# NVlabs/intrinsic3d

Measured on NVIDIA H100. Metric: gauss_newton_iterations_per_sec, higher is better.
Workload: dtype f32

## Files before the change

### intrinsic3d_b200/csrc/i3d_engine.cu

```cuda
#include <cuda_runtime.h>
#include <dlfcn.h>

#include <algorithm>
#include <chrono>
#include <climits>
#include <cmath>
#include <cstdarg>
#include <cstdio>
#include <cstdlib>
#include <cstring>
#include <string>
#include <vector>

#include "../../include/i3d_c_api.h"
#include "i3d_kernels.cuh"
#include "i3d_lighting.cuh"
#include "i3d_recolor.cuh"
#include "i3d_gridops.cuh"
#include "i3d_host.h"
#include "i3d_frames.h"
#include "i3d_fusion.h"
#include "i3d_mesh.h"
#include "i3d_render.h"
#include "i3d_track.h"
// ... 432 lines not shown

int check_frame_limit(I3DEngine* e, int F, int K)
{
    int optin = 0;
    CK(cudaDeviceGetAttribute(&optin, cudaDevAttrMaxSharedMemoryPerBlockOptin, e->device));
    cudaFuncAttributes fa_acc{}, fa_app{};
    CK(cudaFuncGetAttributes(&fa_acc, k_eg_accum));
    CK(cudaFuncGetAttributes(&fa_app, k_eg_apply));
    const size_t lim = static_cast<size_t>(optin);
    auto fits = [&](int f) { return fa_acc.sharedSizeBytes + accum_smem_bytes(f, K) <= lim && fa_app.sharedSizeBytes + apply_smem_bytes(f, K) <= lim; };
    if (fits(F)) return 0;
    int fmax = 0;
    while (fits(fmax + 1)) ++fmax;
    return fail(e, "i3d_gn_iteration: %d frames at K = %d observations need %zu bytes of shared memory per block in k_eg_accum (device limit %d): "
                   "at most %d frames at K = %d", F, K, fa_acc.sharedSizeBytes + accum_smem_bytes(F, K), optin, fmax, K);
}

void launch_eg_apply(I3DEngine* e, const GridView& g, const RegView& rv, const EgRows& rows, const SolveVecs& sv)
{
    if (rows.n_active == 0) return;
    Timer kt(e->timing, e->stream, "k_eg_apply");
    pdl_launch(e, k_eg_apply, blocks_for(rows.n_active), kThreads, apply_smem_bytes(e->F, rows.K), g, rows, rv, sv, sv.ps, e->ctl.p, e->site(SITE_EG_APPLY));
}

void launch_operator(I3DEngine* e, const GridView& g, const RegView& rv, const EgRows& rows, const SolveVecs& sv, const Shard& sh, const float* vin,
                     float dmin, float dmax, int is_cg_iteration)
{
    launch_eg_apply(e, g, rv, rows, sv);
    {
        Timer kt(e->timing, e->stream, "k_op_partial", 1);
        pdl_launch(e, k_op_partial, blocks_for(static_cast<size_t>((e->held_count() + 3) / 4)), kThreads, 0,
            g, rv, sv, sh, e->held_count(), vin, sv.ps, e->type_w.p, dmin, dmax, e->ctl.p, e->site(SITE_OP_POST), e->site(SITE_EG_APPLY).out, is_cg_iteration);
    }
    if (e->world > 1)
    {
        Timer kt(e->timing, e->stream, "exchange", 1);
        exchange(e, sv.qg, nullptr, sv.qg + 2 * e->n, 6 * e->F + 9, e->site(SITE_OP_POST).out, 1, 1, is_cg_iteration ? EPI_OPERATOR_CG : -1);
    }
}

bool plan_cg_step(I3DEngine* e)
{
    if (e->step_n == e->n) return e->step_grid > 0;
    e->step_n = e->n; e->step_grid = 0;
    int sms = 0, optin = 0;
    CK(cudaDeviceGetAttribute(&sms, cudaDevAttrMultiProcessorCount, e->device));
    CK(cudaDeviceGetAttribute(&optin, cudaDevAttrMaxSharedMemoryPerBlockOptin, e->device));
    cudaFuncAttributes fa0{}, fa1{};
    CK(cudaFuncGetAttributes(&fa0, k_cg_step<false>));
    CK(cudaFuncGetAttributes(&fa1, k_cg_step<true>));
    const size_t dyn_max = static_cast<size_t>(optin) - std::max(fa0.sharedSizeBytes, fa1.sharedSizeBytes);
    CK(cudaFuncSetAttribute(k_cg_step<false>, cudaFuncAttributeMaxDynamicSharedMemorySize, static_cast<int>(dyn_max)));
    CK(cudaFuncSetAttribute(k_cg_step<true>, cudaFuncAttributeMaxDynamicSharedMemorySize, static_cast<int>(dyn_max)));
    const int64_t items = (e->n + 3) / 4;
    for (int bps = 2048 / kStepThreads; bps >= 1; --bps)
    {
        const int64_t threads = static_cast<int64_t>(bps) * sms * kStepThreads;
        const int64_t K = (items + threads - 1) / threads;
        const size_t smem = static_cast<size_t>(K) * kStepSlots * kStepThreads * sizeof(float);
        if (smem > dyn_max) break;
        int occ0 = 0, occ1 = 0;
        CK(cudaOccupancyMaxActiveBlocksPerMultiprocessor(&occ0, k_cg_step<false>, kStepThreads, smem));
        CK(cudaOccupancyMaxActiveBlocksPerMultiprocessor(&occ1, k_cg_step<true>, kStepThreads, smem));
        if (std::min(occ0, occ1) < bps) continue;
        if (static_cast<size_t>(bps) * sms + 8 > e->max_blocks) break;
        e->step_grid = static_cast<unsigned>(bps * sms); e->step_K = static_cast<int>(K); e->step_smem = smem;
        return true;
    }
    return false;
}

template <bool INIT>
void launch_cg_step(I3DEngine* e, const GridView& g, const RegView& rv, const SolveVecs& sv, float dmin, float dmax)
{
    const int64_t items = (e->n + 3) / 4;
    pdl_launch<true>(e, k_cg_step<INIT>, e->step_grid, kStepThreads, e->step_smem, g, rv, sv, items, e->step_K, e->type_w.p, e->minv.p, dmin, dmax,
                     e->ctl.p, e->site(SITE_OP_POST), e->site(SITE_EG_APPLY).out, e->site(SITE_UPDATE));
}

int gn_iteration_impl(I3DEngine* e, const I3DParams& P, I3DIterInfo& info)
{
    std::memset(&info, 0, sizeof(info));
    if (e->n <= 0) return fail(e, "i3d_gn_iteration: no grid uploaded");
    if (e->F <= 0) return fail(e, "i3d_gn_iteration: no frames uploaded");
    if (!e->have_cam) return fail(e, "i3d_gn_iteration: camera not set");
    if (!e->have_sh) return fail(e, "i3d_gn_iteration: SH coefficients not set");
    if (e->world > 1 && !e->shard_ready) return fail(e, "i3d_gn_iteration: world > 1 but i3d_set_shard was not called after the grid/frames upload");
    int K = P.num_observations;
    if (K <= 0 || K > e->F) K = e->F;
    if (K > I3D_MAX_OBS) return fail(e, "i3d_gn_iteration: num_observations (%d) exceeds I3D_MAX_OBS (%d)", K, I3D_MAX_OBS);
    if (P.lm_steps < 1) return fail(e, "i3d_gn_iteration: lm_steps < 1");
    if (P.residual_reset_period < 1) return fail(e, "i3d_gn_iteration: residual_reset_period < 1");
    if (check_frame_limit(e, e->F, K) != 0) return 1;
    e->K = K;
    e->last_params = P;
    e->timing.phases.clear(); begin_timing(e->timing, {}); e->launches = 0; e->host_syncs = 0;
    const int64_t n = e->n;
    const int F = e->F;
    const bool multi = e->world > 1;
    cudaStream_t st = e->stream;
    ensure_vectors(e);
    e->iter_dev.ensure(1);
    const Shard sh = e->shard();
    const int64_t own = sh.own_end - sh.own_begin;
    const int64_t hc = e->held_count();
    const size_t U = static_cast<size_t>(e->U());
    Timer t_total(e->timing, e->stream, "total");
    auto sync = [&]() { CK(cudaStreamSynchronize(st)); e->host_syncs += 1; };

    Timer t_sel(e->timing, e->stream, "select");
    e->flags.ensure(n);
    GridView g = e->grid_view(e->sdf, e->alb);
    pdl_launch(e, k_flags, blocks_for(static_cast<size_t>(sh.loc_end - sh.loc_begin)), kThreads, 0, g, sh, P.thres_shell, P.fix_all_albedo, e->flags.p);
    const int nscan = std::max(1, static_cast<int>((own + kScanChunk - 1) / kScanChunk));
    e->scan_counts.ensure(nscan); e->scan_total.ensure(1); e->act.ensure(n);
    pdl_launch(e, k_scan_count, nscan, kThreads, 0, own, e->flags.p + sh.own_begin, FL_ROW, e->scan_counts.p);
    pdl_launch(e, k_scan_blocks, 1, 1024, 0, nscan, e->scan_counts.p, e->scan_total.p);
    pdl_launch(e, k_scan_scatter, nscan, kThreads, 0, own, e->flags.p + sh.own_begin, FL_ROW, e->scan_counts.p, e->act.p, static_cast<int32_t>(sh.own_begin));
    const CamAccLayout lay{F};
    CK(cudaMemsetAsync(e->v_bg.p, 0, U * sizeof(float), st));
    CK(cudaMemsetAsync(e->v_cg.p, 0, U * sizeof(float), st));
    CK(cudaMemsetAsync(e->v_qg.p, 0, U * sizeof(float), st));
    CK(cudaMemsetAsync(e->v_delta.p, 0, U * sizeof(float), st));
    CK(cudaMemsetAsync(e->v_tr.p, 0, static_cast<size_t>(n) * sizeof(float), st));
    CK(cudaMemsetAsync(e->cam_acc.p, 0, lay.size() * sizeof(float), st));
    CK(cudaMemsetAsync(e->v_bgd.p, 0, U * sizeof(double), st));
    CK(cudaMemsetAsync(e->v_cgd.p, 0, U * sizeof(double), st));
    CK(cudaMemsetAsync(e->v_qgd.p, 0, U * sizeof(double), st));
    CK(cudaMemsetAsync(e->cam_accd.p, 0, lay.size() * sizeof(double), st));
    CK(cudaMemsetAsync(e->red_out.p, 0, 2 * kSiteVals * sizeof(double), st));
    e->Rt.ensure(12 * static_cast<size_t>(F));
    e->pose_ctx.ensure(F); e->pose_ctx_c.ensure(F);
    pdl_launch(e, k_pose_mats, blocks_for(F, 64), 64, 0, F, e->cam, e->Rt.p);
    pdl_launch(e, k_frame_pose, blocks_for(F, 64), 64, 0, F, e->cam, e->pose_ctx.p);
    int32_t n_active = 0;
    double hc9[9];
    CK(cudaMemcpyAsync(&n_active, e->scan_total.p, sizeof(int32_t), cudaMemcpyDeviceToHost, st));
    CK(cudaMemcpyAsync(hc9, e->cam + 6 * static_cast<size_t>(F), 9 * sizeof(double), cudaMemcpyDeviceToHost, st));
    sync();
    e->n_active = n_active;
    const int stride = (n_active + 63) & ~63;
    e->stride = stride;
    const size_t S = static_cast<size_t>(K) * stride;

    e->obs_frame.ensure(S + 1); e->obs_w.ensure(S + 1);
    if (n_active > 0)
    {
        const SelectCam sc = select_cam(e, hc9, P.occlusion_distance);
        const size_t smem = 12 * static_cast<size_t>(F) * sizeof(float);
        auto kern = (K <= 5) ? k_select_obs<5> : k_select_obs<I3D_MAX_OBS>;
        if (smem > 48 * 1024) CK(cudaFuncSetAttribute(kern, cudaFuncAttributeMaxDynamicSharedMemorySize, static_cast<int>(smem)));
        Timer kt(e->timing, e->stream, "k_select_obs");
        static const bool want_stats = std::getenv("I3D_CULL_STATS") != nullptr;
        e->cull_stats.ensure(2);
        if (want_stats) CK(cudaMemsetAsync(e->cull_stats.p, 0, 2 * sizeof(unsigned long long), st));
        const CullView cull = cull_view(e, want_stats ? e->cull_stats.p : nullptr);
        pdl_launch(e, kern, blocks_for(static_cast<size_t>(n_active)), kThreads, smem, g, e->frame_view(), e->Rt.p, sc, cull, n_active, stride, e->act.p, K,
                                                                                e->obs_frame.p, e->obs_w.p);
        if (want_stats)
        {
            unsigned long long hs[2] = {0, 0};
            CK(cudaMemcpyAsync(hs, e->cull_stats.p, sizeof(hs), cudaMemcpyDeviceToHost, st));
            CK(cudaStreamSynchronize(st));
            fprintf(stderr, "[i3d] frame culling: %llu of %llu (warp, frame) pairs visited (%.1f %%)\n", hs[0], hs[1], hs[1] ? 100.0 * hs[0] / hs[1] : 0.0);
        }
    }
    t_sel.stop();

    Timer t_build(e->timing, e->stream, "build");
    e->Jt.ensure(EgRows::kTiles * S + 1); e->Jtail.ensure(S + 1);
    e->row_frame.ensure(S + 1); e->row_res.ensure(S + 1); e->row_wraw.ensure(S + 1);
    e->ea_w.ensure(3 * static_cast<size_t>(n)); e->lap.ensure(n);
    CK(cudaFuncSetAttribute(k_eg_apply, cudaFuncAttributeMaxDynamicSharedMemorySize, static_cast<int>(apply_smem_bytes(F, K))));
    const EgRows rows = eg_rows(e);
    CamView cv{e->cam, e->pose_ctx.p, F};
    if (n_active > 0)
    {
        {
            Timer kt(e->timing, e->stream, "k_eg_build");
            launch_eg_rows<ROWS_BUILD>(e, g, cv, rows, e->obs_frame.p, e->obs_w.p);
        }
        const size_t smem = accum_smem_bytes(F, K);
        if (smem > 48 * 1024) CK(cudaFuncSetAttribute(k_eg_accum, cudaFuncAttributeMaxDynamicSharedMemorySize, static_cast<int>(smem)));
        {
            Timer kt(e->timing, e->stream, "k_eg_accum", 1);
            pdl_launch(e, k_eg_accum, blocks_for(static_cast<size_t>(n_active)), kThreads, smem, g, rows, F, e->v_bgd.p, e->v_cgd.p, e->cam_accd.p, e->site(SITE_BUILD));
        }
        pdl_launch(e, k_acc_to_float, blocks_for(std::max(U, static_cast<size_t>(lay.size()))), kThreads, 0, static_cast<int64_t>(U), lay.size(),
                   e->v_bgd.p, e->v_cgd.p, e->cam_accd.p, e->v_bg.p, e->v_cg.p, e->cam_acc.p);
    }
    const RegView rv = reg_view(e, P);
    pdl_launch(e, k_reg_build, blocks_for(static_cast<size_t>((sh.loc_end - sh.loc_begin + 3) / 4)), kThreads, 0, g, rv, sh, e->site(SITE_REG));
    {
        const double na = static_cast<double>(n_active);
        CK(cudaMemcpyAsync(e->site(SITE_BUILD).out + 3, &na, sizeof(double), cudaMemcpyHostToDevice, st));
    }
    if (multi) exchange(e, e->v_bg.p, e->v_cg.p, e->cam_acc.p, lay.size(), e->red_out.p, 2 * kSiteVals, 0);
    pdl_launch(e, k_type_weights, 1, 32, 0, e->iter_dev.p, e->site(SITE_BUILD).out, e->site(SITE_REG).out, P, n, e->type_w.p);
    if (S > 0) pdl_launch(e, k_row_weights, blocks_for(S), kThreads, 0, rows, e->type_w.p);
    SolveVecs sv = solve_vecs(e);
    pdl_launch(e, k_finish_problem, blocks_for(static_cast<size_t>((hc + 3) / 4)), kThreads, 0, g, rv, sv, sh, hc, e->type_w.p, e->cam_acc.p, P.fix_poses, P.fix_intrinsics,
                                                                              P.fix_distortion, P.gradient_tolerance, e->site(SITE_FINISH), e->cam);
    allreduce_scalars(e, e->site(SITE_FINISH).out, 3, -1, 0);
    pdl_launch(e, k_iter_finish, 1, 32, 0, e->iter_dev.p, e->site(SITE_FINISH).out, P);
    t_build.stop();
    e->have_iter = true;
    if (P.build_only)
    {
        IterDev hb{};
        CK(cudaMemcpyAsync(&hb, e->iter_dev.p, sizeof(hb), cudaMemcpyDeviceToHost, st));
        sync();
        CK(cudaGetLastError());
        info = hb.info;
        t_total.stop();
        return 0;
    }

    Timer t_solve(e->timing, e->stream, "solve");
    const float dmin = static_cast<float>(P.min_lm_diagonal), dmax = static_cast<float>(std::min(P.max_lm_diagonal, 3.0e38));
    const unsigned upd_blocks = blocks_for(static_cast<size_t>((sh.held_voxel_unknowns() + 3) / 4 + F + 2));
    auto launch_update = [&](bool init, int refresh) {
        if (init) pdl_launch(e, k_cg_update<true>, upd_blocks, kThreads, 0, sv, sh, e->minv.p, dmin, dmax, e->ctl.p, refresh, e->site(SITE_UPDATE));
        else pdl_launch(e, k_cg_update<false>, upd_blocks, kThreads, 0, sv, sh, e->minv.p, dmin, dmax, e->ctl.p, refresh, e->site(SITE_UPDATE));
    };
    const unsigned vec_blocks = blocks_for(static_cast<size_t>(hc));
    const int max_it = P.forced_cg_iterations > 0 ? P.forced_cg_iterations : P.max_linear_solver_iterations;
    const bool fused = e->pcg_fused && !multi && plan_cg_step(e);
    int enq = 0;
    bool dir_ready = false;
    auto enqueue_pcg = [&](int count) {
        for (int bidx = 0; bidx < count && enq < max_it; ++bidx)
        {
            ++enq;
            const bool refresh = (enq % P.residual_reset_period == 0);
            if (!dir_ready)
            {
                Timer kt(e->timing, e->stream, "k_cg_dir", 1);
                pdl_launch(e, k_cg_dir4, blocks_for(static_cast<size_t>((hc + 3) / 4)), kThreads, 0, sv, sh, hc, e->ctl.p);
            }
            dir_ready = false;
            if (fused && !refresh)
            {
                launch_eg_apply(e, g, rv, rows, sv);
                Timer kt(e->timing, e->stream, "k_cg_update", 1);
                launch_cg_step<false>(e, g, rv, sv, dmin, dmax);
                dir_ready = true;
                continue;
            }
            launch_operator(e, g, rv, rows, sv, sh, sv.p, dmin, dmax, 1);
            if (refresh)
            {
                pdl_launch(e, k_x_update, vec_blocks, kThreads, 0, sv, sh, hc, e->ctl.p);
                CK(cudaMemsetAsync(e->v_qg.p, 0, U * sizeof(float), st));
                pdl_launch(e, k_scale_vec, vec_blocks, kThreads, 0, sv, sh, hc, sv.x, 1.0f, sv.ps, e->ctl.p, 1);
                launch_operator(e, g, rv, rows, sv, sh, sv.x, dmin, dmax, 0);
                launch_update(false, 1);
            }
            else
            {
                Timer kt(e->timing, e->stream, "k_cg_update", 1);
                launch_update(false, 0);
            }
            if (multi) allreduce_scalars(e, e->site(SITE_UPDATE).out, 3, EPI_UPDATE, 1);
        }
    };
    auto enqueue_decision = [&]() {
        Timer t_cand(e->timing, e->stream, "candidate");
        CK(cudaMemsetAsync(e->red_out.p + SITE_CAND * kSiteVals, 0, 3 * kSiteVals * sizeof(double), st));
        pdl_launch(e, k_candidate, vec_blocks, kThreads, 0, g, sv, sh, hc, 0, e->cam, e->c_sdf, e->c_alb, e->c_cam, e->v_delta.p, e->ctl.p, e->site(SITE_CAND));
        GridView gc = e->grid_view(e->c_sdf, e->c_alb);
        pdl_launch(e, k_frame_pose, blocks_for(F, 64), 64, 0, F, e->c_cam, e->pose_ctx_c.p);
        CamView cvc{e->c_cam, e->pose_ctx_c.p, F};
        if (n_active > 0)
        {
            Timer kt(e->timing, e->stream, "k_eg_cost");
            launch_eg_rows<ROWS_COST>(e, gc, cvc, rows, nullptr, nullptr);
        }
        pdl_launch(e, k_reg_cost, blocks_for(static_cast<size_t>(own)), kThreads, 0, gc, rv, sh, e->c_sdf, e->c_alb, e->site(SITE_REG_COST));
        if (multi) allreduce_scalars(e, e->red_out.p + SITE_CAND * kSiteVals, 3 * kSiteVals, -1, 0);
        pdl_launch(e, k_lm_decide, 1, 32, 0, e->iter_dev.p, e->ctl.p, e->fail_flag.p, e->site(SITE_CAND).out, e->site(SITE_EG_COST).out,
                                      e->site(SITE_REG_COST).out, e->type_w.p, P);
    };
    IterDev h{};
    for (int it = 1; it <= P.lm_steps; ++it)
    {
        Timer t_pcg(e->timing, e->stream, "pcg");
        pdl_launch(e, k_lm_begin, 1, 32, 0, e->iter_dev.p, e->ctl.p, e->fail_flag.p, P);
        pdl_launch(e, k_cam_precond, blocks_for(static_cast<size_t>(F) + 2, 64), 64, 0, sv, e->cam_acc.p, e->type_w.p, e->ctl.p, dmin, dmax, e->minv.p, e->fail_flag.p);
        if (fused) launch_cg_step<true>(e, g, rv, sv, dmin, dmax);
        else launch_update(true, 0);
        dir_ready = fused;
        if (multi) allreduce_scalars(e, e->site(SITE_UPDATE).out, 3, EPI_UPDATE_INIT, 0);
        enq = 0;
        enqueue_pcg(P.forced_cg_iterations > 0 ? P.forced_cg_iterations : std::max(e->last_cg_iterations, e->prev_cg_iterations));
        t_pcg.stop();
        while (true)
        {
            enqueue_decision();
            CK(cudaMemcpyAsync(&h, e->iter_dev.p, sizeof(h), cudaMemcpyDeviceToHost, st));
            sync();
            CK(cudaGetLastError());
            if (!h.pcg_unfinished || h.state != LM_RUNNING) break;
            Timer t_more(e->timing, e->stream, "pcg");
            enqueue_pcg(2);
        }
        if (h.info.lm_iterations >= 1)
        {
            e->prev_cg_iterations = e->last_cg_iterations;
            e->last_cg_iterations = std::max(1, h.info.cg_iterations[std::min(h.info.lm_iterations - 1, I3D_MAX_LM_STEPS - 1)]);
        }
        if (h.state != LM_RUNNING) break;
    }
    info = h.info;
    if (h.precond_fail) e->error = "camera preconditioner block not SPD";
    if (h.state == LM_ACCEPTED)
    {
        if (multi)
// ... 1312 lines not shown
```

### intrinsic3d_b200/csrc/i3d_kernels.cuh

```cuda
#pragma once
#include <cuda_runtime.h>
#include <cooperative_groups.h>
#include <stdint.h>
#include <limits.h>
#include "i3d_math.cuh"
#include "i3d_grid.cuh"
#include "../../include/i3d_types.h"

namespace i3d
{

enum : uint8_t { FL_VALID = 1, FL_ACTIVE = 2, FL_RING = 4, FL_FREE_SDF = 8, FL_FREE_ALB = 16, FL_ES_JAC = 32, FL_ROW = 64  };

struct Shard
{
    int64_t own_begin, own_end;
    int64_t hv0, hv1;
    int cam_owner;
    int defer;
    int64_t loc_begin, loc_end;
    __device__ __forceinline__ bool owns_voxel(int64_t v) const { return v >= own_begin && v < own_end; }
    __device__ __forceinline__ bool owns_unknown(int64_t j, int64_t n) const
    {
        return j < n ? owns_voxel(j) : (j < 2 * n ? owns_voxel(j - n) : cam_owner != 0);
// ... 178 lines not shown
}

__global__ void k_flags(GridView g, Shard sh, double thres_shell, int fix_all_albedo, uint8_t* __restrict__ flags)
{
    pdl_prologue();
    const int64_t v = sh.loc_begin + blockIdx.x * static_cast<int64_t>(blockDim.x) + threadIdx.x;
    if (v >= sh.loc_end) return;
    uint8_t fl = 0;
    const bool valid = g.weight[v] > 0.0f;
    if (valid) fl |= FL_VALID;
    bool ring = true;
#pragma unroll
    for (int o = 0; o < 6; ++o)
    {
        const int32_t nb = g.nbr[static_cast<int64_t>(o) * g.n + v];
        if (nb < 0 || !(g.weight[nb] > 0.0f)) ring = false;
    }
    if (ring) fl |= FL_RING;
    const double s = g.sdf[v];
    const bool inshell = !(fabs(s) > thres_shell);
    if (valid && inshell)
    {
        float nrm[3];
        if (surface_normal_f(g, v, nrm)) { fl |= FL_ACTIVE; if (sh.owns_voxel(v)) fl |= FL_ROW; }
        if (ring) { fl |= FL_FREE_SDF; if (!fix_all_albedo) fl |= FL_FREE_ALB; }
    }
    if ((s - g.sdf0[v]) != 0.0) fl |= FL_ES_JAC;
    flags[v] = fl;
}

constexpr int kScanItems = 8;
constexpr int kScanChunk = kThreads * kScanItems;

__global__ void k_scan_count(int64_t n, const uint8_t* __restrict__ flags, uint8_t bit, int32_t* __restrict__ block_counts)
{
    pdl_prologue();
    __shared__ int smem[32];
    const int64_t base = static_cast<int64_t>(blockIdx.x) * kScanChunk;
    int c = 0;
#pragma unroll
    for (int i = 0; i < kScanItems; ++i)
    {
        const int64_t idx = base + static_cast<int64_t>(i) * kThreads + threadIdx.x;
        if (idx < n && (flags[idx] & bit)) c++;
    }
    const int lane = threadIdx.x & 31, wid = threadIdx.x >> 5;
#pragma unroll
    for (int o = 16; o > 0; o >>= 1) c += __shfl_down_sync(0xffffffffu, c, o);
    if (lane == 0) smem[wid] = c;
    __syncthreads();
    if (threadIdx.x == 0)
    {
        int s = 0;
        for (int w = 0; w < kThreads / 32; ++w) s += smem[w];
        block_counts[blockIdx.x] = s;
    }
}

__global__ void k_scan_blocks(int nblocks, int32_t* __restrict__ block_counts, int32_t* __restrict__ total)
{
    pdl_prologue();
    __shared__ int carry;
    __shared__ int wsum[32];
    if (threadIdx.x == 0) carry = 0;
    __syncthreads();
    for (int base = 0; base < nblocks; base += blockDim.x)
    {
        const int i = base + threadIdx.x;
        const int v = (i < nblocks) ? block_counts[i] : 0;
        int incl = v;
        const int lane = threadIdx.x & 31, wid = threadIdx.x >> 5;
#pragma unroll
        for (int o = 1; o < 32; o <<= 1) { const int t = __shfl_up_sync(0xffffffffu, incl, o); if (lane >= o) incl += t; }
        if (lane == 31) wsum[wid] = incl;
        __syncthreads();
        if (wid == 0)
        {
            int w = (lane < (blockDim.x >> 5)) ? wsum[lane] : 0;
#pragma unroll
            for (int o = 1; o < 32; o <<= 1) { const int t = __shfl_up_sync(0xffffffffu, w, o); if (lane >= o) w += t; }
            wsum[lane] = w;
        }
        __syncthreads();
        const int woff = (wid > 0) ? wsum[wid - 1] : 0;
        const int excl = carry + woff + incl - v;
        if (i < nblocks) block_counts[i] = excl;
        __syncthreads();
        if (threadIdx.x == blockDim.x - 1) carry = excl + v;
        __syncthreads();
    }
    if (threadIdx.x == 0) *total = carry;
}

__global__ void k_scan_scatter(int64_t n, const uint8_t* __restrict__ flags, uint8_t bit, const int32_t* __restrict__ block_offsets,
                               int32_t* __restrict__ out_list, int32_t index_offset = 0)
{
    pdl_prologue();
    __shared__ int wsum[kThreads / 32];
    const int64_t base = static_cast<int64_t>(blockIdx.x) * kScanChunk;
    int running = block_offsets[blockIdx.x];
    const int lane = threadIdx.x & 31, wid = threadIdx.x >> 5;
    for (int i = 0; i < kScanItems; ++i)
    {
        const int64_t idx = base + static_cast<int64_t>(i) * kThreads + threadIdx.x;
        const bool f = idx < n && (flags[idx] & bit);
        const unsigned bal = __ballot_sync(0xffffffffu, f);
        if (lane == 0) wsum[wid] = __popc(bal);
        __syncthreads();
        int woff = 0, tot = 0;
        for (int w = 0; w < kThreads / 32; ++w) { const int c = wsum[w]; if (w < wid) woff += c; tot += c; }
        if (f) out_list[running + woff + __popc(bal & ((1u << lane) - 1u))] = static_cast<int32_t>(idx) + index_offset;
        running += tot;
        __syncthreads();
    }
}

__global__ void k_pose_mats(int F, const double* __restrict__ poses, float* __restrict__ Rt )
{
    pdl_prologue();
    const int f = blockIdx.x * blockDim.x + threadIdx.x;
    if (f >= F) return;
    const double wx = poses[6 * f], wy = poses[6 * f + 1], wz = poses[6 * f + 2];
    const double n2 = wx * wx + wy * wy + wz * wz;
    const double angle = sqrt(n2);
    double ax = wx, ay = wy, az = wz;
    if (n2 > 0.0) { ax = wx / angle; ay = wy / angle; az = wz / angle; }
    const double s = sin(angle), c = cos(angle);
    const double sx = __dmul_rn(s, ax), sy = __dmul_rn(s, ay), sz = __dmul_rn(s, az);
    const double c1x = __dmul_rn(1.0 - c, ax), c1y = __dmul_rn(1.0 - c, ay), c1z = __dmul_rn(1.0 - c, az);
    double M[9];
    double tmp;
    tmp = __dmul_rn(c1x, ay); M[1] = tmp - sz; M[3] = tmp + sz;
    tmp = __dmul_rn(c1x, az); M[2] = tmp + sy; M[6] = tmp - sy;
    tmp = __dmul_rn(c1y, az); M[5] = tmp - sx; M[7] = tmp + sx;
    M[0] = __dadd_rn(__dmul_rn(c1x, ax), c); M[4] = __dadd_rn(__dmul_rn(c1y, ay), c); M[8] = __dadd_rn(__dmul_rn(c1z, az), c);
    float* o = Rt + 12 * f;
#pragma unroll
    for (int i = 0; i < 9; ++i) o[i] = static_cast<float>(M[i]);
    o[9] = static_cast<float>(poses[6 * f + 3]); o[10] = static_cast<float>(poses[6 * f + 4]); o[11] = static_cast<float>(poses[6 * f + 5]);
}

__global__ void k_frame_pose(int F, const double* __restrict__ poses, FramePose* __restrict__ out)
{
    pdl_prologue();
    const int f = blockIdx.x * blockDim.x + threadIdx.x;
    if (f >= F) return;
    FramePose fp;
    frame_pose_make(poses + 6 * f, &fp);
    out[f] = fp;
}

struct SelectCam { float fx, fy, cx, cy; float d[5]; int dist_zero; float occlusion; };

__device__ __forceinline__ float observation_weight(const float pt[3], const float nrm[3], const float* __restrict__ Rt, const SelectCam& cam,
                                                    const float* __restrict__ depth, int W, int H, float* pix = nullptr)
{
    float q[3];
#pragma unroll
    for (int k = 0; k < 3; ++k) q[k] = FA(FA(FA(FM(Rt[3 * k], pt[0]), FM(Rt[3 * k + 1], pt[1])), FM(Rt[3 * k + 2], pt[2])), Rt[9 + k]);
    float x = FD(q[0], q[2]);
    float y = FD(q[1], q[2]);
    if (!cam.dist_zero)
    {
        const float r2 = FA(FM(x, x), FM(y, y));
        const float r4 = FM(r2, r2);
        const float r6 = FM(r4, r2);
        const float dc = FA(FA(FA(1.0f, FM(cam.d[0], r2)), FM(cam.d[1], r4)), FM(cam.d[2], r6));
        const float xn = FA(FA(FM(x, dc), FM(FM(FM(2.0f, cam.d[3]), x), y)), FM(cam.d[4], FA(r2, FM(FM(2.0f, x), x))));
        const float yn = FA(FA(FM(y, dc), FM(FM(FM(2.0f, cam.d[4]), xn), y)), FM(cam.d[3], FA(r2, FM(FM(2.0f, y), y))));
        x = xn; y = yn;
    }
    const float pu = FA(FM(cam.fx, x), cam.cx);
    const float pv = FA(FM(cam.fy, y), cam.cy);
    if (pix) { pix[0] = pu; pix[1] = pv; }
    const float pu5 = FA(pu, 0.5f), pv5 = FA(pv, 0.5f);
    if (!(pu5 > -2147483000.0f && pu5 < 2147483000.0f && pv5 > -2147483000.0f && pv5 < 2147483000.0f)) return 0.0f;
    const int iu = __float2int_rz(pu5), iv = __float2int_rz(pv5);
    if (iu < 0 || iu >= W || iv < 0 || iv >= H) return 0.0f;
    const float d = __ldg(depth + static_cast<size_t>(iv) * W + iu);
    if (cam.occlusion > 0.0f)
    {
        if (!(d > 0.0f)) return 0.0f;
        const float sd = FS(d, q[2]);
        if (!(fabsf(sd) <= cam.occlusion)) return 0.0f;
    }
    if (d <= 0.0f) return 0.0f;
    float nc[3];
#pragma unroll
    for (int k = 0; k < 3; ++k) nc[k] = FA(FA(FM(Rt[3 * k], nrm[0]), FM(Rt[3 * k + 1], nrm[1])), FM(Rt[3 * k + 2], nrm[2]));
    float w_normal = 0.0f;
    if (!(nc[0] == 0.0f && nc[1] == 0.0f && nc[2] == 0.0f))
    {
        const float qn2 = FA(FA(FM(q[0], q[0]), FM(q[1], q[1])), FM(q[2], q[2]));
        float v0 = q[0], v1 = q[1], v2 = q[2];
        if (qn2 > 0.0f) { const float ql = __fsqrt_rn(qn2); v0 = FD(q[0], ql); v1 = FD(q[1], ql); v2 = FD(q[2], ql); }
        const float dt = FA(FA(FM(v0, nc[0]), FM(v1, nc[1])), FM(v2, nc[2]));
        w_normal = FS(1.0f, fabsf(dt));
        w_normal = (1.0f < w_normal) ? 1.0f : w_normal;
        w_normal = (w_normal < 0.0f) ? 0.0f : w_normal;
        const float div = FA(1.0f, FM(2.0f, w_normal));
        const float rk = FD(1.0f, FM(FM(div, div), div));
        w_normal = (rk < 0.001f) ? 0.001f : rk;
    }
    return w_normal;
}

struct ObsProbe { float q0, q1, q2, d; int ok; };
__device__ __forceinline__ ObsProbe obs_probe(const float pt[3], const float* __restrict__ Rt, const SelectCam& cam, const float* __restrict__ depth, int W, int H)
{
    ObsProbe o;
    float q[3];
#pragma unroll
    for (int k = 0; k < 3; ++k) q[k] = FA(FA(FA(FM(Rt[3 * k], pt[0]), FM(Rt[3 * k + 1], pt[1])), FM(Rt[3 * k + 2], pt[2])), Rt[9 + k]);
    o.q0 = q[0]; o.q1 = q[1]; o.q2 = q[2]; o.d = 0.0f; o.ok = 0;
    float x = FD(q[0], q[2]);
    float y = FD(q[1], q[2]);
    if (!cam.dist_zero)
    {
        const float r2 = FA(FM(x, x), FM(y, y));
        const float r4 = FM(r2, r2);
        const float r6 = FM(r4, r2);
        const float dc = FA(FA(FA(1.0f, FM(cam.d[0], r2)), FM(cam.d[1], r4)), FM(cam.d[2], r6));
        const float xn = FA(FA(FM(x, dc), FM(FM(FM(2.0f, cam.d[3]), x), y)), FM(cam.d[4], FA(r2, FM(FM(2.0f, x), x))));
        const float yn = FA(FA(FM(y, dc), FM(FM(FM(2.0f, cam.d[4]), xn), y)), FM(cam.d[3], FA(r2, FM(FM(2.0f, y), y))));
        x = xn; y = yn;
    }
    const float pu5 = FA(FA(FM(cam.fx, x), cam.cx), 0.5f), pv5 = FA(FA(FM(cam.fy, y), cam.cy), 0.5f);
    if (!(pu5 > -2147483000.0f && pu5 < 2147483000.0f && pv5 > -2147483000.0f && pv5 < 2147483000.0f)) return o;
    const int iu = __float2int_rz(pu5), iv = __float2int_rz(pv5);
    if (iu < 0 || iu >= W || iv < 0 || iv >= H) return o;
    o.d = __ldg(depth + static_cast<size_t>(iv) * W + iu);
    o.ok = 1;
    return o;
}
__device__ __forceinline__ float obs_finish(const ObsProbe& o, const float nrm[3], const float* __restrict__ Rt, const SelectCam& cam)
{
    if (!o.ok) return 0.0f;
    const float d = o.d;
    const float q[3] = {o.q0, o.q1, o.q2};
    if (cam.occlusion > 0.0f)
    {
        if (!(d > 0.0f)) return 0.0f;
        const float sd = FS(d, q[2]);
        if (!(fabsf(sd) <= cam.occlusion)) return 0.0f;
    }
    if (d <= 0.0f) return 0.0f;
    float nc[3];
#pragma unroll
    for (int k = 0; k < 3; ++k) nc[k] = FA(FA(FM(Rt[3 * k], nrm[0]), FM(Rt[3 * k + 1], nrm[1])), FM(Rt[3 * k + 2], nrm[2]));
    float w_normal = 0.0f;
    if (!(nc[0] == 0.0f && nc[1] == 0.0f && nc[2] == 0.0f))
    {
        const float qn2 = FA(FA(FM(q[0], q[0]), FM(q[1], q[1])), FM(q[2], q[2]));
        float v0 = q[0], v1 = q[1], v2 = q[2];
        if (qn2 > 0.0f) { const float ql = __fsqrt_rn(qn2); v0 = FD(q[0], ql); v1 = FD(q[1], ql); v2 = FD(q[2], ql); }
        const float dt = FA(FA(FM(v0, nc[0]), FM(v1, nc[1])), FM(v2, nc[2]));
        w_normal = FS(1.0f, fabsf(dt));
        w_normal = (1.0f < w_normal) ? 1.0f : w_normal;
        w_normal = (w_normal < 0.0f) ? 0.0f : w_normal;
        const float div = FA(1.0f, FM(2.0f, w_normal));
        const float rk = FD(1.0f, FM(FM(div, div), div));
        w_normal = (rk < 0.001f) ? 0.001f : rk;
    }
    return w_normal;
}

constexpr int kCullTile = 32;
constexpr int kCullMaxWords = 16;

__global__ void k_depth_tiles(int F, int W, int H, const float* __restrict__ depth, float* __restrict__ tmin, float* __restrict__ tmax)
{
    const int TW = (W + kCullTile - 1) / kCullTile, TH = (H + kCullTile - 1) / kCullTile;
    const int t = blockIdx.x;
    if (t >= F * TW * TH) return;
    const int f = t / (TW * TH), r = t % (TW * TH), ty = r / TW, tx = r % TW;
    const float* img = depth + static_cast<size_t>(f) * W * H;
    float mn = __int_as_float(0x7f800000), mx = 0.0f;
    for (int i = threadIdx.x; i < kCullTile * kCullTile; i += blockDim.x)
    {
        const int px = tx * kCullTile + (i % kCullTile), py = ty * kCullTile + (i / kCullTile);
        if (px < W && py < H)
        {
            const float d = img[static_cast<size_t>(py) * W + px];
            if (d > 0.0f) { mn = fminf(mn, d); mx = fmaxf(mx, d); }
        }
    }
#pragma unroll
    for (int o = 16; o > 0; o >>= 1) { mn = fminf(mn, __shfl_xor_sync(0xffffffffu, mn, o)); mx = fmaxf(mx, __shfl_xor_sync(0xffffffffu, mx, o)); }
    __shared__ float smn[8], smx[8];
    if ((threadIdx.x & 31) == 0) { smn[threadIdx.x >> 5] = mn; smx[threadIdx.x >> 5] = mx; }
    __syncthreads();
    if (threadIdx.x == 0)
    {
        for (int w = 1; w < (blockDim.x >> 5); ++w) { mn = fminf(mn, smn[w]); mx = fmaxf(mx, smx[w]); }
        tmin[t] = mn; tmax[t] = mx;
    }
}

struct CullView { const float* tmin; const float* tmax; int enabled; unsigned long long* stats;  };

__device__ __forceinline__ bool frame_may_see(const float c[3], float rad, const float* __restrict__ Rt, const SelectCam& cam, const CullView& cv,
                                              int f, int W, int H)
{
    const float qx = Rt[0] * c[0] + Rt[1] * c[1] + Rt[2] * c[2] + Rt[9];
    const float qy = Rt[3] * c[0] + Rt[4] * c[1] + Rt[5] * c[2] + Rt[10];
    const float qz = Rt[6] * c[0] + Rt[7] * c[1] + Rt[8] * c[2] + Rt[11];
    const float zmin = qz - rad, zmax = qz + rad;
    if (!(zmin > 1e-3f)) return true;
    const float iz = 1.0f / qz;
    float xc = qx * iz, yc = qy * iz;
    const float rnx = rad * (1.0f + fabsf(xc)) / zmin, rny = rad * (1.0f + fabsf(yc)) / zmin;
    float lip = 1.0f;
    if (!cam.dist_zero)
    {
        const float R = sqrtf(xc * xc + yc * yc) + 1.4143f * fmaxf(rnx, rny);
        const float R2 = R * R;
        const float grow = 3.0f * fabsf(cam.d[0]) * R2 + 5.0f * fabsf(cam.d[1]) * R2 * R2 + 7.0f * fabsf(cam.d[2]) * R2 * R2 * R2 +
                           8.0f * (fabsf(cam.d[3]) + fabsf(cam.d[4])) * R;
        lip = 1.0f + 2.0f * grow * (1.0f + 2.0f * fabsf(cam.d[4]) * R);
        const float r2 = xc * xc + yc * yc;
        const float dc = 1.0f + cam.d[0] * r2 + cam.d[1] * r2 * r2 + cam.d[2] * r2 * r2 * r2;
        const float xd = xc * dc + 2.0f * cam.d[3] * xc * yc + cam.d[4] * (r2 + 2.0f * xc * xc);
        const float yd = yc * dc + 2.0f * cam.d[4] * xd * yc + cam.d[3] * (r2 + 2.0f * yc * yc);
        xc = xd; yc = yd;
    }
    const float uc = cam.fx * xc + cam.cx, vc = cam.fy * yc + cam.cy;
    const float ru = cam.fx * 1.4143f * fmaxf(rnx, rny) * lip * 1.001f + 2.0f;
    const float rv = cam.fy * 1.4143f * fmaxf(rnx, rny) * lip * 1.001f + 2.0f;
    if (uc + ru < 0.0f || uc - ru > static_cast<float>(W) || vc + rv < 0.0f || vc - rv > static_cast<float>(H)) return false;
    const int TW = (W + kCullTile - 1) / kCullTile, TH = (H + kCullTile - 1) / kCullTile;
    const int tx0 = max(0, static_cast<int>(floorf((uc - ru) / kCullTile))), tx1 = min(TW - 1, static_cast<int>(floorf((uc + ru) / kCullTile)));
    const int ty0 = max(0, static_cast<int>(floorf((vc - rv) / kCullTile))), ty1 = min(TH - 1, static_cast<int>(floorf((vc + rv) / kCullTile)));
    if (tx1 - tx0 > 3 || ty1 - ty0 > 3) return true;
    float dmin = __int_as_float(0x7f800000), dmax = 0.0f;
    const float* mn = cv.tmin + static_cast<size_t>(f) * TW * TH;
    const float* mx = cv.tmax + static_cast<size_t>(f) * TW * TH;
    for (int ty = ty0; ty <= ty1; ++ty)
        for (int tx = tx0; tx <= tx1; ++tx) { dmin = fminf(dmin, mn[ty * TW + tx]); dmax = fmaxf(dmax, mx[ty * TW + tx]); }
    if (!(dmax > 0.0f)) return false;
    if (cam.occlusion > 0.0f)
    {
        const float tol = cam.occlusion * 1.001f + 1e-4f;
        if (zmin > dmax + tol || zmax < dmin - tol) return false;
    }
    return true;
}

template <int KMAX>
__global__ void __launch_bounds__(kThreads)
k_select_obs(GridView g, FrameView fr, const float* __restrict__ Rt, SelectCam cam, CullView cull, int n_active, int stride,
             const int32_t* __restrict__ act, int K, int32_t* __restrict__ obs_frame , float* __restrict__ obs_w )
{
    pdl_prologue();
    extern __shared__ float s_rt[];
    for (int i = threadIdx.x; i < 12 * fr.F; i += blockDim.x) s_rt[i] = Rt[i];
    __syncthreads();
    const int lane = threadIdx.x & 31;
    const int a = blockIdx.x * blockDim.x + threadIdx.x;
    const bool in_range = a < n_active;
    if (__ballot_sync(0xffffffffu, in_range) == 0u) return;
    float nrm[3] = {0.0f, 0.0f, 0.0f};
    float pt[3] = {0.0f, 0.0f, 0.0f};
    if (in_range)
    {
        const int64_t v = act[a];
        surface_normal_f(g, v, nrm);
        const float s = static_cast<float>(g.sdf[v]);
        pt[0] = FS(FM(static_cast<float>(g.x[v]), g.voxel_size), FM(nrm[0], s));
        pt[1] = FS(FM(static_cast<float>(g.y[v]), g.voxel_size), FM(nrm[1], s));
        pt[2] = FS(FM(static_cast<float>(g.z[v]), g.voxel_size), FM(nrm[2], s));
    }
    const int nwords = (fr.F + 31) / 32;
    __shared__ unsigned s_mask[kThreads / 32][kCullMaxWords];
    unsigned* wmask = s_mask[threadIdx.x >> 5];
    const bool culling = cull.enabled && nwords <= kCullMaxWords;
    if (culling)
    {
        const float big = 3.0e38f;
        float lo[3], hi[3];
#pragma unroll
        for (int k = 0; k < 3; ++k) { lo[k] = in_range ? pt[k] : big; hi[k] = in_range ? pt[k] : -big; }
#pragma unroll
        for (int o = 16; o > 0; o >>= 1)
#pragma unroll
            for (int k = 0; k < 3; ++k) { lo[k] = fminf(lo[k], __shfl_xor_sync(0xffffffffu, lo[k], o)); hi[k] = fmaxf(hi[k], __shfl_xor_sync(0xffffffffu, hi[k], o)); }
        const float c[3] = {0.5f * (lo[0] + hi[0]), 0.5f * (lo[1] + hi[1]), 0.5f * (lo[2] + hi[2])};
        const float dx = hi[0] - lo[0], dy = hi[1] - lo[1], dz = hi[2] - lo[2];
        const float rad = 0.5f * sqrtf(dx * dx + dy * dy + dz * dz) * 1.001f + 1e-4f;
#pragma unroll 1
        for (int j = 0; j < nwords; ++j)
        {
            const int f = 32 * j + lane;
            const bool may = (f < fr.F) && frame_may_see(c, rad, s_rt + 12 * f, cam, cull, f, fr.W, fr.H);
            const unsigned m = __ballot_sync(0xffffffffu, may);
            if (lane == 0) wmask[j] = m;
        }
        __syncwarp();
    }
    const size_t img = static_cast<size_t>(fr.W) * fr.H;
    unsigned long long best[KMAX];
#pragma unroll
    for (int k = 0; k < KMAX; ++k) best[k] = 0ull;
    auto insert = [&](float wf, int f) {
        if (wf > 0.0f && in_range)
        {
            unsigned long long key = (static_cast<unsigned long long>(__float_as_uint(wf)) << 32) | static_cast<unsigned>(f + 1);
#pragma unroll
            for (int k = 0; k < KMAX; ++k)
            {
                const unsigned long long hi2 = key > best[k] ? key : best[k];
                const unsigned long long lo2 = key > best[k] ? best[k] : key;
                best[k] = hi2; key = lo2;
            }
        }
    };
    if (cull.stats && lane == 0)
    {
        unsigned long long vis = 0;
        for (int j = 0; j < nwords; ++j) vis += culling ? __popc(wmask[j]) : 32;
        atomicAdd(cull.stats, vis); atomicAdd(cull.stats + 1, static_cast<unsigned long long>(fr.F));
    }
    ObsProbe pend; pend.ok = 0; pend.q0 = pend.q1 = pend.q2 = pend.d = 0.0f;
    int pend_f = -1;
#pragma unroll 1
    for (int j = 0; j < nwords; ++j)
    {
        unsigned m = culling ? wmask[j] : 0xffffffffu;
#pragma unroll 1
        while (m)
        {
            const int f = 32 * j + __ffs(m) - 1;
            m &= m - 1;
            if (f >= fr.F) continue;
            const ObsProbe nxt = obs_probe(pt, s_rt + 12 * f, cam, fr.depth + img * f, fr.W, fr.H);
            if (pend_f >= 0) insert(obs_finish(pend, nrm, s_rt + 12 * pend_f, cam), pend_f);
            pend = nxt; pend_f = f;
        }
    }
    if (pend_f >= 0) insert(obs_finish(pend, nrm, s_rt + 12 * pend_f, cam), pend_f);
    if (!in_range) return;
#pragma unroll
    for (int k = 0; k < KMAX; ++k)
    {
        if (k >= K || best[k] == 0ull) best[k] = ~0ull;
        else best[k] = ((best[k] & 0xffffffffull) << 32) | (best[k] >> 32);
    }
#pragma unroll
    for (int i = 0; i < KMAX; ++i)
#pragma unroll
        for (int j = 0; j + 1 < KMAX - i; ++j)
        {
            const unsigned long long lo = best[j] < best[j + 1] ? best[j] : best[j + 1];
            const unsigned long long hi = best[j] < best[j + 1] ? best[j + 1] : best[j];
            best[j] = lo; best[j + 1] = hi;
        }
#pragma unroll
    for (int k = 0; k < KMAX; ++k)
    {
        if (k >= K) break;
        int fsel = -1; float wsel = 0.0f;
        if (best[k] != ~0ull) { fsel = static_cast<int>(best[k] >> 32) - 1; wsel = __uint_as_float(static_cast<unsigned>(best[k] & 0xffffffffull)); }
        obs_frame[static_cast<size_t>(k) * stride + a] = fsel;
        obs_w[static_cast<size_t>(k) * stride + a] = wsel;
    }
}

struct CamView
{
    const double* cam;
    const FramePose* fpose;
    int F;
};

struct EgRows
{
    int n_active, K;
    int stride;
    const int32_t* act;
    float4* Jt;
    float2* Jtail;
    int32_t* row_frame;
    double* row_res;
    double* row_wraw;
    static constexpr int kTiles = 7;
    __host__ __device__ size_t slots() const { return static_cast<size_t>(K) * stride; }
    __device__ __forceinline__ void store_row(size_t slot, const float row[29]) const
    {
        const size_t S = slots();
#pragma unroll
        for (int c = 0; c < kTiles; ++c) Jt[c * S + slot] = make_float4(row[4 * c], row[4 * c + 1], row[4 * c + 2], row[4 * c + 3]);
        Jtail[slot].x = row[28];
    }
    template <bool STREAM>
    __device__ __forceinline__ float load_row(size_t slot, float jr[29]) const
    {
        const size_t S = slots();
#pragma unroll
        for (int c = 0; c < kTiles; ++c)
        {
            const float4 t = STREAM ? __ldcs(Jt + c * S + slot) : Jt[c * S + slot];
            jr[4 * c] = t.x; jr[4 * c + 1] = t.y; jr[4 * c + 2] = t.z; jr[4 * c + 3] = t.w;
        }
        const float2 t = STREAM ? __ldcs(Jtail + slot) : Jtail[slot];
        jr[28] = t.x;
        return t.y;
    }
};

__device__ __forceinline__ void make_cam_params(const CamView& cv, double pyr_scale, int W, int H, CamParams<double>* c)
{
    const double* intr = cv.cam + 6 * cv.F;
    const double* dist = intr + 4;
    c->fx = intr[0] * pyr_scale; c->fy = intr[1] * pyr_scale; c->cx = intr[2] * pyr_scale; c->cy = intr[3] * pyr_scale;
    c->k1 = dist[0]; c->k2 = dist[1]; c->k3 = dist[2]; c->p1 = dist[3]; c->p2 = dist[4];
    c->pyr_scale = pyr_scale; c->w = W; c->h = H;
}

__device__ __forceinline__ bool gather_stencil(const GridView& g, const double* __restrict__ sdf, const double* __restrict__ alb, int64_t v,
                                               int32_t idx[14], double s10[10], double a4[4])
{
    const int64_t n = g.n;
    const int32_t xp = g.nbr[NB_XP * n + v], yp = g.nbr[NB_YP * n + v], zp = g.nbr[NB_ZP * n + v];
    const int32_t x2 = g.nbr[NB_X2 * n + v], y2 = g.nbr[NB_Y2 * n + v], z2 = g.nbr[NB_Z2 * n + v];
    const int32_t xy = g.nbr[NB_XY * n + v], xz = g.nbr[NB_XZ * n + v], yz = g.nbr[NB_YZ * n + v];
    idx[0] = static_cast<int32_t>(v); idx[1] = yp; idx[2] = y2; idx[3] = yz; idx[4] = zp; idx[5] = z2; idx[6] = xp; idx[7] = xy; idx[8] = xz; idx[9] = x2;
    idx[10] = static_cast<int32_t>(v); idx[11] = xp; idx[12] = yp; idx[13] = zp;
    bool ok = true;
#pragma unroll
    for (int k = 0; k < 10; ++k) ok = ok && (idx[k] >= 0);
    if (!ok) return false;
#pragma unroll
    for (int k = 0; k < 10; ++k) s10[k] = sdf[idx[k]];
#pragma unroll
    for (int k = 0; k < 4; ++k) a4[k] = alb[idx[10 + k]];
    return true;
}

__device__ __forceinline__ double sdf_to_weight(double sdf, double truncation)
{
    const double a = fmin(fabs(sdf), truncation) / truncation;
    return fmin(fmax(1.0 - a, 0.01), 1.0);
}

struct CamAccLayout
{
    int F;
    __host__ __device__ int pose_stride() const { return 33; }
    __host__ __device__ int tail() const { return 33 * F; }
    __host__ __device__ int size() const { return 33 * F + 43; }
};

enum { ROWS_BUILD = 0, ROWS_COST = 1 };
constexpr int kRowThreads = 128;

__device__ __forceinline__ uint32_t smem_u32(const void* p) { return static_cast<uint32_t>(__cvta_generic_to_shared(p)); }
__device__ __forceinline__ void mbar_init(uint64_t* bar, uint32_t count)
{
    asm volatile("mbarrier.init.shared::cta.b64 [%0], %1;" ::"r"(smem_u32(bar)), "r"(count) : "memory");
    asm volatile("fence.mbarrier_init.release.cluster;" ::: "memory");
}
__device__ __forceinline__ void mbar_expect_tx(uint64_t* bar, uint32_t bytes)
{
    asm volatile("mbarrier.arrive.expect_tx.shared::cta.b64 _, [%0], %1;" ::"r"(smem_u32(bar)), "r"(bytes) : "memory");
}
__device__ __forceinline__ void bulk_copy_g2s(void* dst_smem, const void* src_gmem, uint32_t bytes , uint64_t* bar)
{
    asm volatile("cp.async.bulk.shared::cluster.global.mbarrier::complete_tx::bytes [%0], [%1], %2, [%3];"
                 ::"r"(smem_u32(dst_smem)), "l"(src_gmem), "r"(bytes), "r"(smem_u32(bar)) : "memory");
}
__device__ __forceinline__ void mbar_wait(uint64_t* bar, uint32_t parity)
{
    uint32_t done = 0;
    while (!done)
        asm volatile("{\n\t.reg .pred P1;\n\tmbarrier.try_wait.parity.shared::cta.b64 P1, [%1], %2;\n\tselp.b32 %0, 1, 0, P1;\n\t}"
                     : "=r"(done) : "r"(smem_u32(bar)), "r"(parity) : "memory");
}

static_assert(kVoxelGeomWords == 15, "VoxelGeom size changed: update the pose-table staging boundary and its test");
__host__ __device__ inline size_t rows_pose_bytes(int F) { return (static_cast<size_t>(F) * sizeof(FramePose) + 127) & ~static_cast<size_t>(127); }
__host__ __device__ inline size_t rows_smem_bytes(int mode, int threads, bool stage, int F)
{
    return (stage ? 128 + rows_pose_bytes(F) : 0) + static_cast<size_t>(threads) * (kVoxelGeomWords * sizeof(double) + (mode == ROWS_BUILD ? kVoxelDerivWords * sizeof(float) : 0));
}

template <int MODE, int THREADS, bool STAGE>
__global__ void __launch_bounds__(THREADS, THREADS == 128 ? 4 : 2)
k_eg_rows(GridView g, FrameView fr, CamView cv, EgRows rows, const int32_t* __restrict__ obs_frame, const float* __restrict__ obs_w, ReduceSite site)
{
    extern __shared__ __align__(128) unsigned char s_rows[];
    pdl_prologue();
    uint64_t* s_bar = reinterpret_cast<uint64_t*>(s_rows);
    const FramePose* s_pose = reinterpret_cast<const FramePose*>(s_rows + 128);
// ... 1646 lines not shown
```

Before: 140.5.

## Order frame probes by view-angle buckets and skip frames that cannot enter top-K

In the observation-selection kernel, visible frames are now grouped per warp into angle buckets, so frames with a likely high normal weight are probed first. A per-thread rejection bound, derived from the current K-th best weight, skips the depth lookup and full weight evaluation when the view angle cannot beat that weight, and a frame is skipped entirely when the whole warp rejects it. The block size drops to 128 threads with a min-blocks launch bound. The bucketing adds shuffle and ballot work plus larger shared masks, and the bound relies on careful float margins to keep the selection exact.

```diff
diff --git a/intrinsic3d_b200/csrc/i3d_engine.cu b/intrinsic3d_b200/csrc/i3d_engine.cu
--- a/intrinsic3d_b200/csrc/i3d_engine.cu
+++ b/intrinsic3d_b200/csrc/i3d_engine.cu
@@ -608,17 +608,18 @@
         if (smem > 48 * 1024) CK(cudaFuncSetAttribute(kern, cudaFuncAttributeMaxDynamicSharedMemorySize, static_cast<int>(smem)));
         Timer kt(e->timing, e->stream, "k_select_obs");
         static const bool want_stats = std::getenv("I3D_CULL_STATS") != nullptr;
-        e->cull_stats.ensure(2);
-        if (want_stats) CK(cudaMemsetAsync(e->cull_stats.p, 0, 2 * sizeof(unsigned long long), st));
+        e->cull_stats.ensure(3);
+        if (want_stats) CK(cudaMemsetAsync(e->cull_stats.p, 0, 3 * sizeof(unsigned long long), st));
         const CullView cull = cull_view(e, want_stats ? e->cull_stats.p : nullptr);
-        pdl_launch(e, kern, blocks_for(static_cast<size_t>(n_active)), kThreads, smem, g, e->frame_view(), e->Rt.p, sc, cull, n_active, stride, e->act.p, K,
+        pdl_launch(e, kern, blocks_for(static_cast<size_t>(n_active), kSelectThreads), kSelectThreads, smem, g, e->frame_view(), e->Rt.p, sc, cull, n_active, stride, e->act.p, K,
                                                                                 e->obs_frame.p, e->obs_w.p);
         if (want_stats)
         {
-            unsigned long long hs[2] = {0, 0};
+            unsigned long long hs[3] = {0, 0, 0};
             CK(cudaMemcpyAsync(hs, e->cull_stats.p, sizeof(hs), cudaMemcpyDeviceToHost, st));
             CK(cudaStreamSynchronize(st));
-            fprintf(stderr, "[i3d] frame culling: %llu of %llu (warp, frame) pairs visited (%.1f %%)\n", hs[0], hs[1], hs[1] ? 100.0 * hs[0] / hs[1] : 0.0);
+            fprintf(stderr, "[i3d] frame culling: %llu of %llu (warp, frame) pairs visited (%.1f %%), %llu with the full weight (%.1f %%)\n",
+                    hs[0], hs[1], hs[1] ? 100.0 * hs[0] / hs[1] : 0.0, hs[2], hs[1] ? 100.0 * hs[2] / hs[1] : 0.0);
         }
     }
     t_sel.stop();
diff --git a/intrinsic3d_b200/csrc/i3d_kernels.cuh b/intrinsic3d_b200/csrc/i3d_kernels.cuh
--- a/intrinsic3d_b200/csrc/i3d_kernels.cuh
+++ b/intrinsic3d_b200/csrc/i3d_kernels.cuh
@@ -354,6 +354,16 @@
 
 struct SelectCam { float fx, fy, cx, cy; float d[5]; int dist_zero; float occlusion; };
 
+__device__ __forceinline__ float normal_weight(float adt)
+{
+    float w_normal = FS(1.0f, adt);
+    w_normal = (1.0f < w_normal) ? 1.0f : w_normal;
+    w_normal = (w_normal < 0.0f) ? 0.0f : w_normal;
+    const float div = FA(1.0f, FM(2.0f, w_normal));
+    const float rk = FD(1.0f, FM(FM(div, div), div));
+    return (rk < 0.001f) ? 0.001f : rk;
+}
+
 __device__ __forceinline__ float observation_weight(const float pt[3], const float nrm[3], const float* __restrict__ Rt, const SelectCam& cam,
                                                     const float* __restrict__ depth, int W, int H, float* pix = nullptr)
 {
@@ -397,24 +407,17 @@
         float v0 = q[0], v1 = q[1], v2 = q[2];
         if (qn2 > 0.0f) { const float ql = __fsqrt_rn(qn2); v0 = FD(q[0], ql); v1 = FD(q[1], ql); v2 = FD(q[2], ql); }
         const float dt = FA(FA(FM(v0, nc[0]), FM(v1, nc[1])), FM(v2, nc[2]));
-        w_normal = FS(1.0f, fabsf(dt));
-        w_normal = (1.0f < w_normal) ? 1.0f : w_normal;
-        w_normal = (w_normal < 0.0f) ? 0.0f : w_normal;
-        const float div = FA(1.0f, FM(2.0f, w_normal));
-        const float rk = FD(1.0f, FM(FM(div, div), div));
-        w_normal = (rk < 0.001f) ? 0.001f : rk;
+        w_normal = normal_weight(fabsf(dt));
     }
     return w_normal;
 }
 
 struct ObsProbe { float q0, q1, q2, d; int ok; };
-__device__ __forceinline__ ObsProbe obs_probe(const float pt[3], const float* __restrict__ Rt, const SelectCam& cam, const float* __restrict__ depth, int W, int H)
+__device__ __forceinline__ ObsProbe obs_probe(const float q[3], bool want, const SelectCam& cam, const float* __restrict__ depth, int W, int H)
 {
     ObsProbe o;
-    float q[3];
-#pragma unroll
-    for (int k = 0; k < 3; ++k) q[k] = FA(FA(FA(FM(Rt[3 * k], pt[0]), FM(Rt[3 * k + 1], pt[1])), FM(Rt[3 * k + 2], pt[2])), Rt[9 + k]);
     o.q0 = q[0]; o.q1 = q[1]; o.q2 = q[2]; o.d = 0.0f; o.ok = 0;
+    if (!want) return o;
     float x = FD(q[0], q[2]);
     float y = FD(q[1], q[2]);
     if (!cam.dist_zero)
@@ -457,14 +460,25 @@
         float v0 = q[0], v1 = q[1], v2 = q[2];
         if (qn2 > 0.0f) { const float ql = __fsqrt_rn(qn2); v0 = FD(q[0], ql); v1 = FD(q[1], ql); v2 = FD(q[2], ql); }
         const float dt = FA(FA(FM(v0, nc[0]), FM(v1, nc[1])), FM(v2, nc[2]));
-        w_normal = FS(1.0f, fabsf(dt));
-        w_normal = (1.0f < w_normal) ? 1.0f : w_normal;
-        w_normal = (w_normal < 0.0f) ? 0.0f : w_normal;
-        const float div = FA(1.0f, FM(2.0f, w_normal));
-        const float rk = FD(1.0f, FM(FM(div, div), div));
-        w_normal = (rk < 0.001f) ? 0.001f : rk;
+        w_normal = normal_weight(fabsf(dt));
     }
     return w_normal;
+}
+
+__device__ __forceinline__ float topk_reject_const(unsigned tau_bits)
+{
+    if (tau_bits == 0u) return 0.0f;
+    const float tau = __uint_as_float(tau_bits);
+    const float c0 = 0.5f * (3.0f - rcbrtf(tau)) - 0x1p-14f;
+    if (!(c0 > 0x1p-15f) || !(normal_weight(c0) < tau)) return 0.0f;
+    const float c1 = c0 - 0x1p-16f;
+    return c1 * c1;
+}
+__device__ __forceinline__ bool topk_rejects(const float q[3], const float nc[3], float C)
+{
+    const float qn2 = FA(FA(FM(q[0], q[0]), FM(q[1], q[1])), FM(q[2], q[2]));
+    const float a = q[0] * nc[0] + q[1] * nc[1] + q[2] * nc[2];
+    return qn2 >= 0x1p-60f && qn2 <= 0x1p100f && a * a < C * qn2;
 }
 
 constexpr int kCullTile = 32;
@@ -548,8 +562,11 @@
     return true;
 }
 
+constexpr int kObsBuckets = 8;
+__constant__ float kObsBucketCos2[kObsBuckets - 1] = {0.9801f, 0.9409f, 0.9025f, 0.8464f, 0.7225f, 0.5625f, 0.36f};
+constexpr int kSelectThreads = 128;
 template <int KMAX>
-__global__ void __launch_bounds__(kThreads)
+__global__ void __launch_bounds__(kSelectThreads, 1024 / kSelectThreads)
 k_select_obs(GridView g, FrameView fr, const float* __restrict__ Rt, SelectCam cam, CullView cull, int n_active, int stride,
              const int32_t* __restrict__ act, int K, int32_t* __restrict__ obs_frame , float* __restrict__ obs_w )
 {
@@ -573,19 +590,23 @@
         pt[2] = FS(FM(static_cast<float>(g.z[v]), g.voxel_size), FM(nrm[2], s));
     }
     const int nwords = (fr.F + 31) / 32;
-    __shared__ unsigned s_mask[kThreads / 32][kCullMaxWords];
-    unsigned* wmask = s_mask[threadIdx.x >> 5];
+    __shared__ unsigned s_mask[kSelectThreads / 32][kObsBuckets][kCullMaxWords];
+    unsigned (*wmask)[kCullMaxWords] = s_mask[threadIdx.x >> 5];
     const bool culling = cull.enabled && nwords <= kCullMaxWords;
     if (culling)
     {
         const float big = 3.0e38f;
-        float lo[3], hi[3];
-#pragma unroll
-        for (int k = 0; k < 3; ++k) { lo[k] = in_range ? pt[k] : big; hi[k] = in_range ? pt[k] : -big; }
+        float lo[3], hi[3], nm[3];
+#pragma unroll
+        for (int k = 0; k < 3; ++k) { lo[k] = in_range ? pt[k] : big; hi[k] = in_range ? pt[k] : -big; nm[k] = nrm[k]; }
 #pragma unroll
         for (int o = 16; o > 0; o >>= 1)
 #pragma unroll
-            for (int k = 0; k < 3; ++k) { lo[k] = fminf(lo[k], __shfl_xor_sync(0xffffffffu, lo[k], o)); hi[k] = fmaxf(hi[k], __shfl_xor_sync(0xffffffffu, hi[k], o)); }
+            for (int k = 0; k < 3; ++k)
+            {
+                lo[k] = fminf(lo[k], __shfl_xor_sync(0xffffffffu, lo[k], o)); hi[k] = fmaxf(hi[k], __shfl_xor_sync(0xffffffffu, hi[k], o));
+                nm[k] += __shfl_xor_sync(0xffffffffu, nm[k], o);
+            }
         const float c[3] = {0.5f * (lo[0] + hi[0]), 0.5f * (lo[1] + hi[1]), 0.5f * (lo[2] + hi[2])};
         const float dx = hi[0] - lo[0], dy = hi[1] - lo[1], dz = hi[2] - lo[2];
         const float rad = 0.5f * sqrtf(dx * dx + dy * dy + dz * dz) * 1.001f + 1e-4f;
@@ -594,8 +615,29 @@
         {
             const int f = 32 * j + lane;
             const bool may = (f < fr.F) && frame_may_see(c, rad, s_rt + 12 * f, cam, cull, f, fr.W, fr.H);
-            const unsigned m = __ballot_sync(0xffffffffu, may);
-            if (lane == 0) wmask[j] = m;
+            int bucket = kObsBuckets - 1;
+            if (may)
+            {
+                const float* R = s_rt + 12 * f;
+                float qc[3], nr[3];
+#pragma unroll
+                for (int k = 0; k < 3; ++k)
+                {
+                    qc[k] = R[3 * k] * c[0] + R[3 * k + 1] * c[1] + R[3 * k + 2] * c[2] + R[9 + k];
+                    nr[k] = R[3 * k] * nm[0] + R[3 * k + 1] * nm[1] + R[3 * k + 2] * nm[2];
+                }
+                const float dn = qc[0] * nr[0] + qc[1] * nr[1] + qc[2] * nr[2];
+                const float qq = (qc[0] * qc[0] + qc[1] * qc[1] + qc[2] * qc[2]) * (nr[0] * nr[0] + nr[1] * nr[1] + nr[2] * nr[2]);
+#pragma unroll
+                for (int b = kObsBuckets - 2; b >= 0; --b)
+                    if (dn * dn >= kObsBucketCos2[b] * qq) bucket = b;
+            }
+#pragma unroll
+            for (int b = 0; b < kObsBuckets; ++b)
+            {
+                const unsigned m = __ballot_sync(0xffffffffu, may && bucket == b);
+                if (lane == 0) wmask[b][j] = m;
+            }
         }
         __syncwarp();
     }
@@ -616,30 +658,62 @@
             }
         }
     };
-    if (cull.stats && lane == 0)
-    {
-        unsigned long long vis = 0;
-        for (int j = 0; j < nwords; ++j) vis += culling ? __popc(wmask[j]) : 32;
-        atomicAdd(cull.stats, vis); atomicAdd(cull.stats + 1, static_cast<unsigned long long>(fr.F));
-    }
+    const bool bound_on = cull.enabled && in_range &&
+                          fabsf(nrm[0] * nrm[0] + nrm[1] * nrm[1] + nrm[2] * nrm[2] - 1.0f) <= 0x1p-20f;
+    float rej_c = 0.0f;
+    unsigned tau_seen = 0u;
+    auto finish = [&](const ObsProbe& o, int f) {
+        insert(obs_finish(o, nrm, s_rt + 12 * f, cam), f);
+        if (bound_on)
+        {
+            unsigned tau = 0u;
+#pragma unroll
+            for (int k = 0; k < KMAX; ++k) if (k == K - 1) tau = static_cast<unsigned>(best[k] >> 32);
+            if (tau != tau_seen) { tau_seen = tau; rej_c = topk_reject_const(tau); }
+        }
+    };
     ObsProbe pend; pend.ok = 0; pend.q0 = pend.q1 = pend.q2 = pend.d = 0.0f;
     int pend_f = -1;
+    unsigned n_full = 0;
+#pragma unroll 1
+    for (int b = 0; b < (culling ? kObsBuckets : 1); ++b)
 #pragma unroll 1
     for (int j = 0; j < nwords; ++j)
     {
-        unsigned m = culling ? wmask[j] : 0xffffffffu;
+        unsigned m = culling ? wmask[b][j] : 0xffffffffu;
 #pragma unroll 1
         while (m)
         {
             const int f = 32 * j + __ffs(m) - 1;
             m &= m - 1;
             if (f >= fr.F) continue;
-            const ObsProbe nxt = obs_probe(pt, s_rt + 12 * f, cam, fr.depth + img * f, fr.W, fr.H);
-            if (pend_f >= 0) insert(obs_finish(pend, nrm, s_rt + 12 * pend_f, cam), pend_f);
+            const float* R = s_rt + 12 * f;
+            float q[3], nc[3];
+#pragma unroll
+            for (int k = 0; k < 3; ++k)
+            {
+                q[k] = FA(FA(FA(FM(R[3 * k], pt[0]), FM(R[3 * k + 1], pt[1])), FM(R[3 * k + 2], pt[2])), R[9 + k]);
+                nc[k] = FA(FA(FM(R[3 * k], nrm[0]), FM(R[3 * k + 1], nrm[1])), FM(R[3 * k + 2], nrm[2]));
+            }
+            const bool want = in_range && !topk_rejects(q, nc, rej_c);
+            if (__ballot_sync(0xffffffffu, want) == 0u) continue;
+            ++n_full;
+            const ObsProbe nxt = obs_probe(q, want, cam, fr.depth + img * f, fr.W, fr.H);
+            if (pend_f >= 0) finish(pend, pend_f);
             pend = nxt; pend_f = f;
         }
     }
-    if (pend_f >= 0) insert(obs_finish(pend, nrm, s_rt + 12 * pend_f, cam), pend_f);
+    if (pend_f >= 0) finish(pend, pend_f);
+    if (cull.stats && lane == 0)
+    {
+        unsigned long long vis = 0;
+        for (int j = 0; j < nwords; ++j)
+        {
+            if (!culling) { vis += 32; continue; }
+            for (int b = 0; b < kObsBuckets; ++b) vis += __popc(wmask[b][j]);
+        }
+        atomicAdd(cull.stats, vis); atomicAdd(cull.stats + 1, static_cast<unsigned long long>(fr.F)); atomicAdd(cull.stats + 2, static_cast<unsigned long long>(n_full));
+    }
     if (!in_range) return;
 #pragma unroll
     for (int k = 0; k < KMAX; ++k)
```

Result: faster. 142.7 (median of 6 runs) (+1.5%).
